# nschejtman/deepLoopCloser

Measured on AMD Instinct MI355X. Metric: query-frames/sec vs N-keyframe DB + top-k recall@1, higher is better.
Workload: dtype bf16; 1 GPU; 1000000 x 4096 bf16 keyframe DB, Q=256, top-20 cosine match, 1 GPU(s); db_rows=1000000, dim=4096, k=20, rows_per_gpu=1000000, pipelined=False, crowded=False

## Files before the change

deeploopcloser_amd/_lib.py:

```python
import ctypes as C
import os

_HERE = os.path.dirname(os.path.abspath(__file__))
LIB_PATH = os.path.join(_HERE, "libdlc_hip.so")

DLC_OK = 0
DLC_ERR_BAD_ARG, DLC_ERR_BAD_SHAPE, DLC_ERR_UNSUPPORTED, DLC_ERR_HIP, DLC_ERR_WORKSPACE = -1, -2, -3, -4, -5
DLC_BF16, DLC_F16, DLC_F32, DLC_F64, DLC_I8, DLC_U8, DLC_I64 = 0, 1, 2, 3, 4, 5, 6
DLC_ACT_NONE, DLC_ACT_SIGMOID, DLC_ACT_RELU = 0, 1, 2
DLC_B_KN, DLC_B_NK = 0, 1
DLC_MAX_K = 128
DLC_MAX_STEP = 8
DLC_MAX_SHIFT = 8
DLC_ABI_VERSION = 20
DLC_SELECT_COOP, DLC_SELECT_NO_HINTS, DLC_SELECT_SERIAL = 1, 2, 4
DLC_PRUNE_ON, DLC_PRUNE_OFF, DLC_PRUNE_KEEP = 0, 1, 2
DLC_SIM_FORCE_F64, DLC_SIM_NO_HOST_SYNC = 1, 2
DLC_MAX_FUSE = 8
DLC_FUSE_NONE, DLC_FUSE_ZSCORE, DLC_FUSE_MINMAX = 0, 1, 2
DLC_FUSE_PLAN_AUTO, DLC_FUSE_PLAN_ROW, DLC_FUSE_PLAN_SLAB = 0, 1, 2
DLC_TRACK_AUTO, DLC_TRACK_RESIDENT, DLC_TRACK_ROWS = 0, 1, 2
DLC_TRACK_RESIDENT_MAX = 8192
DLC_TRACK_JUMP, DLC_TRACK_FROM_NULL, DLC_TRACK_ORIGIN, DLC_TRACK_ABSENT = -1, -2, -3, -128
DLC_TRACK_END_FILTERED, DLC_TRACK_NO_PATH = -2, -2
# ... 104 lines not shown
    "dlc_pca_project_workspace_bytes": (_sz, [_i64, _i64, _int, _int]),
    "dlc_pca_project": (_int, [_vp, _vp, _i64, _i64, _i64, _vp, _int, _vp, _int, _i64, _vp, _vp, _i64, _int, _vp, _sz, _vp]),
    "dlc_pr_cell_counts_workspace_bytes": (_sz, [_i64, _i64, _int]),
    "dlc_pr_cell_counts": (_int, [_vp, _int, _vp, _i64, _i64, _i64, _i64, _i64, _int, _int, _i64, _vp, _i64, _vp, _int, _vp, _vp,
                                  _vp, _sz, _vp]),
    "dlc_positive_rank_rows_workspace_bytes": (_sz, [_i64, _i64]),
    "dlc_positive_rank_rows": (_int, [_vp, _int, _vp, _i64, _i64, _i64, _i64, _i64, _int, _int, _i64, _vp, _i64, _vp, _vp, _vp,
                                      _vp, _sz, _vp]),
    "dlc_l2_normalize_rows": (_int, [_vp, _int, _vp, _i64, _i64, _i64, _int, _int, _vp, _i64, _vp]),
    "dlc_cosine_topk_workspace_bytes": (_sz, [_i64, _i64, _i64, _int]),
    "dlc_cosine_topk": (_int, [_vp, _int, _vp, _i64, _i64, _vp, _i64, _i64, _i64, _int, _i64, _vp, _vp, _vp, _vp, _vp, _vp, _sz,
                              _vp]),
    "dlc_max_row_norm": (_int, [_vp, _int, _vp, _i64, _i64, _i64, _vp, _vp]),
    "dlc_cosine_tau_scale": (_int, [_vp, _int, _vp, _i64, _i64, _i64, _vp, _vp, _vp]),
    "dlc_cosine_topk_older": (_int, [_vp, _int, _vp, _i64, _i64, _vp, _i64, _i64, _i64, _int, _i64, _i64, _vp, _vp, _vp, _vp, _vp,
                                    _vp, _sz, _vp]),
    "dlc_cosine_score_error_bound": (_dbl, [_i64, _i64, _i64, _int]),
    "dlc_cosine_score_error_bound_any_plan": (_dbl, [_i64]),
    "dlc_cosine_score_groups": (_int, [_vp, _int, _vp, _i64, _i64, _vp, _i64, _i64, _i64, _int, _vp, _sz, _vp]),
    "dlc_cosine_select_topk": (_int, [_vp, _int, _vp, _i64, _i64, _vp, _i64, _i64, _i64, _int, _i64, _vp, _vp, _vp, _vp, _vp, _vp,
                                     _sz, _int, _vp]),
    "dlc_cosine_groups_per_query": (_int, [_int]),
    "dlc_cosine_select_groups": (_int, [_vp, _int, _vp, _i64, _i64, _vp, _i64, _i64, _i64, _int, _vp, _sz, _vp, _vp, _int,
                                       _vp]),
    "dlc_cosine_rescore_topk": (_int, [_vp, _int, _vp, _i64, _i64, _vp, _i64, _i64, _i64, _int, _i64, _vp, _vp, _vp, _int,
                                      _vp, _vp, _vp, _vp, _int, _vp]),
    "dlc_cosine_exhaustive_topk": (_int, [_vp, _int, _vp, _i64, _i64, _vp, _i64, _i64, _i64, _int, _i64, _vp, _i64, _dbl,
                                         _vp, _vp, _vp, _vp, _vp, _vp, _sz, _vp]),
    "dlc_topk_merge_strided": (_int, [_vp, _vp, _i64, _vp, _i64, _int, _i64, _int, _vp, _dbl, _vp, _vp, _vp, _vp, _vp, _vp]),
    "dlc_topk_merge": (_int, [_vp, _vp, _vp, _int, _i64, _int, _vp, _vp, _vp, _vp]),
    "dlc_topk_keep_older": (_int, [_vp, _vp, _vp, _i64, _int, _i64, _int, _vp, _vp, _vp]),
    "dlc_cosine_scores_workspace_bytes": (_sz, [_i64, _i64, _i64]),
    "dlc_cosine_scores": (_int, [_vp, _int, _vp, _i64, _i64, _vp, _i64, _i64, _i64, _vp, _i64, _vp, _sz, _vp]),
    "dlc_cosine_score_rows": (_int, [_vp, _int, _vp, _i64, _i64, _vp, _i64, _i64, _i64, _i64, _i64, _vp, _vp, _i64, _vp]),
    "dlc_host_to_device": (_int, [_vp, _vp, _vp, _sz, _vp]),
    "dlc_device_to_host": (_int, [_vp, _vp, _vp, _sz, _vp]),
    "dlc_set_host_threads": (_int, [_vp, _int]),
    "dlc_set_scratch": (_int, [_vp, _vp, _sz]),
    "dlc_set_profiling": (_int, [_vp, _int]),
    "dlc_set_prune_mode": (_int, [_vp, _int]),
    "dlc_cosine_topk_prune_bytes": (_sz, [_i64, _i64, _i64, _int]),
    "dlc_profile_gemm_ms": (_int, [_vp, C.POINTER(_flt), _int]),
}

_lib = None


class DlcError(RuntimeError):
    """A HIP-side failure (DLC_ERR_HIP / DLC_ERR_WORKSPACE) reported by the C ABI."""


def load():
    global _lib
    if _lib is not None:
        return _lib
    if not os.path.exists(LIB_PATH):
        raise ImportError(
            "deeploopcloser_amd: %s is missing -- build it with `python -c 'import __graft_entry__ as g; g.build()'` "
            "or `make -C deeploopcloser_amd/csrc`.  There is no CPU fallback." % LIB_PATH)
    lib = C.CDLL(LIB_PATH)
    for name, (res, args) in SIGNATURES.items():
        fn = getattr(lib, name)
        fn.restype = res
        fn.argtypes = args
    if lib.dlc_abi_version() != DLC_ABI_VERSION:
        raise ImportError("deeploopcloser_amd: %s has ABI %d, these bindings are for ABI %d -- rebuild it"
# ... 14 lines not shown
```

deeploopcloser_amd/csrc/cosine_topk.hip:

```cpp
#include "dlc_internal.h"
#include "lds_dma.h"

#include <algorithm>

namespace {

constexpr int BM = 256;
constexpr int BNQ = 256;
constexpr int BK = 64;
constexpr int NTHREADS = 512;
constexpr int TILE_BYTES = 256 * BK * 2;
constexpr int A_TILE = TILE_BYTES;
constexpr int B_TILE = TILE_BYTES;
#ifndef DLC_A_STAGES
#define DLC_A_STAGES 2
#endif
constexpr int A_STAGES = DLC_A_STAGES;
constexpr int B_RING = A_STAGES * A_TILE;
constexpr int LDS_BYTES = A_STAGES * A_TILE + 2 * B_TILE;
#ifndef DLC_STAGGER_SLEEP
#define DLC_STAGGER_SLEEP 15
#endif
#ifndef DLC_STAGGER_PHASES
#define DLC_STAGGER_PHASES 32
// ... 48 lines not shown
struct alignas(8) HintEntry {
    float r2;
    int id;
};

struct GemmArgs {
    const char* Q;
    const char* DB;
    long long ldq_b;
    long long lddb_b;
    int q;
    long long n;
    int nk;
    float* gmax;
    long long ldg;
    float* tmax;
    long long ldt;
    HintEntry* hint;
    long long ng;
    long long nh;
    float* S;
    long long lds;
    int stagger_mult;
    int stagger_phases;
    int nqb;
    long long ntiles;
    int nsplit;
    int kchunk;
    float* P;
    long long ldp;
    unsigned* bkt;
    unsigned* thr;
    int kt;
};

constexpr int GEMM_GROUPS = 0;
constexpr int GEMM_DENSE = 1;
constexpr int GEMM_PARTIAL = 2;

constexpr int HALF_BYTES = 128 * 128;

#ifndef DLC_A_CACHE_POLICY
#define DLC_A_CACHE_POLICY " nt"
#endif
DLC_DMA_S_FORM(dma_s_stream, DLC_A_CACHE_POLICY)

constexpr int tail_vmcnt_a(int left) {
    const int whole = (left < A_STAGES - 1 ? left : A_STAGES - 1) - 1;
    return 8 * (whole > 0 ? whole : 0) + (left >= A_STAGES ? 4 : 0);
}
constexpr int tail_vmcnt_b(int left) { return left >= 2 ? 8 : 0; }
static_assert(A_STAGES == 2 || A_STAGES == 3, "the database ring is 2 or 3 K tiles deep");
static_assert(A_STAGES != 2 || (tail_vmcnt_a(2) == 4 && tail_vmcnt_a(1) == 0 && tail_vmcnt_a(0) == 0), "2-deep A ring");
static_assert(A_STAGES != 3 || (tail_vmcnt_a(3) == 12 && tail_vmcnt_a(2) == 8 && tail_vmcnt_a(1) == 0 && tail_vmcnt_a(0) == 0),
              "3-deep A ring");

template <typename Tag, int MODE, bool MASKQ>
__global__ __launch_bounds__(NTHREADS, 2) void score_gemm_kernel(GemmArgs p) {
    extern __shared__ __attribute__((aligned(16))) char smem[];
    const int tid = threadIdx.x;
    const int lane = tid & 63;
    const int wid = __builtin_amdgcn_readfirstlane(tid >> 6);
    const int wr = wid >> 2;
    const int wc = wid & 3;
    const unsigned chunk = MODE == GEMM_PARTIAL ? blockIdx.x % (unsigned)p.nsplit : 0u;
    const unsigned wg = MODE == GEMM_PARTIAL ? blockIdx.x / (unsigned)p.nsplit : blockIdx.x;
    const unsigned run = 8u * (unsigned)p.nqb;
    const int j_ = (int)(wg % run);
    const long long tile = (long long)(wg / run) * 8 + (j_ & 7);
    const int qblk = j_ >> 3;
    if (tile >= p.ntiles) return;
    const unsigned lds_base = (unsigned)(unsigned long long)(lptr_t)smem;

    const bool is_a = wid < 4;
    const int ridx = wid & 3;
    const int k_begin = MODE == GEMM_PARTIAL ? (int)chunk * p.kchunk : 0;
    const char* a_base = p.DB + tile * BM * p.lddb_b + (long long)k_begin * 128;
    const char* b_base = p.Q + (long long)qblk * BNQ * p.ldq_b + (long long)k_begin * 128;
    unsigned voff[2][4];
    {
        const int slot = lane & 7;
        const long long arows = p.n - tile * BM;
        const long long brows = (long long)p.q - (long long)qblk * BNQ;
#pragma unroll
        for (int j = 0; j < 4; ++j) {
            const int r = 32 * ridx + 8 * j + (lane >> 3);
#pragma unroll
            for (int h = 0; h < 2; ++h) {
                long long ar = (r >> 6) * 128 + h * 64 + (r & 63);
                if (ar > arows - 1) ar = arows - 1;
                long long br = (r >> 5) * 64 + h * 32 + (r & 31);
                if (br > brows - 1) br = brows - 1;
                voff[h][j] = is_a ? (unsigned)(ar * p.lddb_b + ((slot ^ swz_a(r)) << 4))
                                  : (unsigned)(br * p.ldq_b + ((slot ^ swz_b(r)) << 4));
            }
        }
    }
    const unsigned lds_stage = lds_base + (unsigned)(32 * ridx) * 128;
    const int nk = MODE == GEMM_PARTIAL ? min(p.kchunk, p.nk - k_begin) : p.nk;

    const int i = lane & 15;
    const int kq = lane >> 4;
    const int fa = ((i >> 1) & 1) | ((i >> 2) << 1);
    const int fb = (i >> 1) & 7;
    typedef const __attribute__((address_space(3))) u32x4_t* lds_u4p;
    const lcptr_t lbase = (lcptr_t)(lptr_t)smem;
    const unsigned rdA0_l = (wr * 64 + 16 * (i >> 2) + (i & 3)) * 128 + (((0 + kq) ^ fa) << 4);
    const unsigned rdA1_l = (wr * 64 + 16 * (i >> 2) + (i & 3)) * 128 + (((4 + kq) ^ fa) << 4);
    const unsigned rdB0_l = B_RING + (wc * 32 + i) * 128 + (((0 + kq) ^ fb) << 4);
    const unsigned rdB1_l = B_RING + (wc * 32 + i) * 128 + (((4 + kq) ^ fb) << 4);
    unsigned aoff = 0, boff = 0;
    unsigned rdA0 = rdA0_l, rdA1 = rdA1_l, rdB0 = rdB0_l, rdB1 = rdB1_l;

    f32x4_t acc[8][4];
#pragma unroll
    for (int t = 0; t < 8; ++t)
#pragma unroll
        for (int c = 0; c < 4; ++c) acc[t][c] = (f32x4_t){0.f, 0.f, 0.f, 0.f};
    u32x4_t faX[4], faY[4], fbX[2], fbY[2];

    const bool active = !MASKQ || (qblk * BNQ + wc * 64 < p.q);
#define DLC_READ_A(DST, RD, OFF)                      \
    if (!MASKQ || active) _Pragma("unroll") for (int tt = 0; tt < 4; ++tt)  \
        DST[tt] = *(lds_u4p)(lbase + (RD) + (OFF) + tt * 512)
#define DLC_READ_B(DST, RD, OFF)                      \
    if (!MASKQ || active) _Pragma("unroll") for (int c = 0; c < 2; ++c)     \
        DST[c] = *(lds_u4p)(lbase + (RD) + (OFF) + c * 2048)
#define DLC_MFMA(FA, FB, AH, BH)                                                                     \
    if (!MASKQ || active) do {                                                                       \
        __builtin_amdgcn_s_setprio(1);                                                               \
        _Pragma("unroll") for (int tt = 0; tt < 4; ++tt) _Pragma("unroll") for (int c = 0; c < 2; ++c) \
            acc[(AH) * 4 + tt][(BH) * 2 + c] =                                                       \
                Mfma16<Tag>::run(FA[tt], FB[c], acc[(AH) * 4 + tt][(BH) * 2 + c]);                   \
        __builtin_amdgcn_s_setprio(0);                                                               \
    } while (0)
#define DLC_RELEASE()    \
    DLC_WAIT_LGKM0();    \
    wg_barrier()
#define DLC_ISSUE_A(POS, H, t2)                                                                      \
    do {                                                                                             \
        if (is_a)                                                                                    \
            dma_s_stream(voff[H], a_base + (long long)(t2) * 128, lds_stage + (POS) + (H) * HALF_BYTES); \
    } while (0)
    const bool b_on = !MASKQ || (qblk * BNQ + ridx * 64 < p.q);
#define DLC_ISSUE_B(POS, H, t2)                                                                      \
    do {                                                                                             \
        if (!is_a && b_on)                                                                           \
            dma_s(voff[H], b_base + (long long)(t2) * 128, lds_stage + B_RING + (POS) + (H) * HALF_BYTES); \
    } while (0)
#define DLC_WAIT_TILE(L)                                                                             \
    do {                                                                                             \
        if constexpr (tail_vmcnt_a(L) == tail_vmcnt_b(L)) DLC_WAIT_VMCNT(tail_vmcnt_a(L));           \
        else if (is_a) DLC_WAIT_VMCNT(tail_vmcnt_a(L));                                              \
        else DLC_WAIT_VMCNT(tail_vmcnt_b(L));                                                        \
    } while (0)

    if (MODE != GEMM_PARTIAL && wg < 256) {
        const int steps = (int)((tile >> 3) % p.stagger_phases) * p.stagger_mult;
        for (int s_ = 0; s_ < steps; ++s_) __builtin_amdgcn_s_sleep(DLC_STAGGER_SLEEP);
    }
#pragma unroll
    for (int s_ = 0; s_ < A_STAGES; ++s_) {
        if (s_ < nk) {
            DLC_ISSUE_A(s_ * A_TILE, 1, s_);
            DLC_ISSUE_A(s_ * A_TILE, 0, s_);
        }
    }
    DLC_ISSUE_B(0 * B_TILE, 0, 0);
    DLC_ISSUE_B(0 * B_TILE, 1, 0);
    if (nk > 1) {
        DLC_ISSUE_B(1 * B_TILE, 0, 1);
        DLC_ISSUE_B(1 * B_TILE, 1, 1);
    }
    if (nk == 1) DLC_WAIT_VMCNT(0);
    else if (A_STAGES == 3 && is_a && nk > 2) DLC_WAIT_VMCNT(16);
    else DLC_WAIT_VMCNT(8);
    wg_barrier();
    DLC_READ_A(faX, rdA0, 0);
    DLC_READ_B(fbX, rdB0, 0);

#define DLC_K_TILE(L)                                                                                \
    do {                                                                                             \
        DLC_READ_B(fbY, rdB0, HALF_BYTES);                                                           \
        DLC_MFMA(faX, fbX, 0, 0);                                                            \
        DLC_READ_A(faY, rdA0, HALF_BYTES);                                                           \
        DLC_MFMA(faX, fbY, 0, 1);                                                            \
        DLC_READ_A(faX, rdA1, HALF_BYTES);                                                           \
        DLC_MFMA(faY, fbY, 1, 1);                                                            \
        DLC_RELEASE();                                                      \
        DLC_READ_B(fbY, rdB1, 0);                                                                    \
        if constexpr ((L) >= A_STAGES) DLC_ISSUE_A(aoff, 1, t + A_STAGES);                           \
        DLC_MFMA(faY, fbX, 1, 0);                                                            \
        DLC_RELEASE();                                                                       \
        DLC_READ_B(fbX, rdB1, HALF_BYTES);                                                           \
        if constexpr ((L) >= 2) DLC_ISSUE_B(boff, 0, t + 2);                                         \
        DLC_MFMA(faX, fbY, 1, 0);                                                            \
        DLC_RELEASE();                                                                       \
        DLC_READ_A(faY, rdA1, 0);                                                                    \
        if constexpr ((L) >= 2) DLC_ISSUE_B(boff, 1, t + 2);                                         \
        DLC_MFMA(faX, fbX, 1, 1);                                                            \
        DLC_WAIT_TILE(L);                                           \
        DLC_RELEASE();                                               \
        if constexpr ((L) >= A_STAGES) DLC_ISSUE_A(aoff, 0, t + A_STAGES);                           \
        aoff = aoff == (A_STAGES - 1) * A_TILE ? 0u : aoff + A_TILE;    \
        boff ^= B_TILE;                                                                              \
        rdA0 = rdA0_l + aoff; rdA1 = rdA1_l + aoff; rdB0 = rdB0_l + boff; rdB1 = rdB1_l + boff;      \
        DLC_READ_A(faX, rdA0, 0);                                                                    \
        DLC_MFMA(faY, fbX, 0, 1);                                                            \
        DLC_READ_B(fbX, rdB0, 0);                                                                    \
        DLC_MFMA(faY, fbY, 0, 0);                                                            \
        ++t;                                                                                         \
    } while (0)
    static_assert(tail_vmcnt_a(1) == 0 && tail_vmcnt_b(1) == 0 && tail_vmcnt_a(0) == 0 && tail_vmcnt_b(0) == 0 && A_STAGES >= 2,
                  "DLC_K_TILE(1) serves L = 0 too");
    int t = 0;
    while (t < nk - A_STAGES) DLC_K_TILE(A_STAGES);
    if constexpr (A_STAGES == 3) {
        if (nk > 2) DLC_K_TILE(2);
    }
#pragma unroll 1
    while (t < nk) DLC_K_TILE(1);
    DLC_WAIT_VMCNT(0);
    DLC_WAIT_LGKM0();
#undef DLC_K_TILE
#undef DLC_WAIT_TILE
#undef DLC_ISSUE_A
#undef DLC_ISSUE_B
#undef DLC_READ_A
#undef DLC_READ_B
#undef DLC_MFMA
#undef DLC_RELEASE

    const int lg = lane >> 4;
    if constexpr (MODE == GEMM_PARTIAL) {
        float* part = p.P + (long long)chunk * p.q * p.ldp;
#pragma unroll
        for (int c = 0; c < 4; ++c) {
            const int qidx = qblk * BNQ + wc * 64 + c * 16 + i;
            if (qidx >= p.q) continue;
#pragma unroll
            for (int t = 0; t < 8; ++t) {
                const long long row0 = tile * BM + wr * 128 + (t >> 2) * 64 + 16 * lg + 4 * (t & 3);
                *(f32x4_t*)(part + (long long)qidx * p.ldp + row0) = acc[t][c];
            }
        }
    } else if constexpr (MODE == GEMM_DENSE) {
#pragma unroll
        for (int c = 0; c < 4; ++c) {
// ... 1634 lines not shown
    return w.prune_total - w.total;
}

namespace {

struct MatchCall {
    GemmArgs a;
    WsLayout w;
    bool publish_thr = false;
};

int prepare_match(dlc_ctx* ctx, const char* what, int dtype, const void* Q, int64_t q, int64_t ldq, const void* DB,
                  int64_t n, int64_t lddb, int64_t d, int k, void* workspace, size_t workspace_bytes, MatchCall* mc) {
    int rc = check_operands(ctx, dtype, Q, q, ldq, DB, n, lddb, d);
    if (rc != DLC_OK) return rc;
    if (k < 1 || k > DLC_MAX_K) return dlc::fail(ctx, DLC_ERR_BAD_ARG, "%s: k=%d outside 1..%d", what, k, DLC_MAX_K);
    mc->w = ws_layout(q, n, d, k);
    if (!workspace || workspace_bytes < mc->w.total)
        return dlc::fail(ctx, DLC_ERR_WORKSPACE, "%s: workspace %zu < %zu bytes", what, workspace_bytes, mc->w.total);
    if (((uintptr_t)workspace & 255)) return dlc::fail(ctx, DLC_ERR_BAD_ARG, "%s: workspace must be 256-byte aligned", what);
    char* ws = (char*)workspace;
    GemmArgs& a = mc->a;
    a.Q = (const char*)Q; a.DB = (const char*)DB;
    a.ldq_b = ldq * 2; a.lddb_b = lddb * 2;
    a.q = (int)q; a.n = n; a.nk = (int)(d / BK);
    a.gmax = (float*)(ws + mc->w.gmax); a.ldg = mc->w.ldg;
    a.tmax = (float*)(ws + mc->w.tmax); a.ldt = mc->w.ldt;
    a.hint = (HintEntry*)(ws + mc->w.hint);
    a.ng = dlc::cdiv(n, GROUP); a.nh = dlc::cdiv(n, HALF);
    a.S = nullptr; a.lds = 0;
    a.nsplit = mc->w.sp.nsplit; a.kchunk = mc->w.sp.kchunk;
    a.P = (float*)(ws + mc->w.part); a.ldp = mc->w.ldp;
    a.bkt = nullptr; a.thr = nullptr; a.kt = 0;
    return DLC_OK;
}

inline bool small_direct(const MatchCall& mc, int k) {
    return mc.w.dense && mc.a.n <= (int64_t)FIN_THREADS * SMALL_GPT * GROUP && k + DENSE_ROW_SLACK + 1 <= SMALL_KT_MAX;
}

int run_score(dlc_ctx* ctx, int dtype, MatchCall& mc, hipStream_t st, bool partials_only = false) {
    return dlc::profiled(ctx, st, [&]() -> int {
        return (dtype == DLC_BF16) ? launch_scores<dlc_bf16_tag>(ctx, mc.a, false, st, mc.w.dense, partials_only)
                                   : launch_scores<dlc_f16_tag>(ctx, mc.a, false, st, mc.w.dense, partials_only);
    });
}

FinishArgs finish_args(const MatchCall& mc, int k, int64_t n, int64_t d, int64_t q, int64_t row_offset) {
    const GemmArgs& g = mc.a;
    FinishArgs f{};
    f.tmax = g.tmax; f.ldt = g.ldt; f.nh = (int)g.nh;
    f.gmax = g.gmax; f.ldg = g.ldg; f.ng = g.ng;
    f.kg = mc.w.kg;
    f.Q = g.Q; f.ldq_b = g.ldq_b; f.DB = g.DB; f.lddb_b = g.lddb_b;
    f.n = n; f.d = (int)d; f.k = k; f.row_offset = row_offset;
    f.tau = mc.w.tau;
    f.nq = q;
    return f;
}

template <typename Tag, int THREADS, int RS_UNROLL, int MODE>
int launch_finish(dlc_ctx* ctx, FinishArgs f, int64_t q, bool small_lds, hipStream_t st) {
    size_t dsm = fin_lds_fixed(f.kg);
    f.tv_in_lds = MODE != FIN_RESCORE && !small_lds && !fin_register_path(THREADS, MODE == FIN_GROUPS, f.nh) &&
                  (size_t)f.nh * 4 <= FIN_TV_LDS_MAX;
    if (f.tv_in_lds) dsm += (size_t)f.nh * 4;
    dsm = dlc::align_up(dsm, 16);
    void (*fk)(FinishArgs);
    if constexpr (THREADS == 256) fk = finish_topk_coop_kernel<Tag, RS_UNROLL, MODE>;
    else fk = finish_topk_kernel<Tag, THREADS, RS_UNROLL, MODE>;
    if (dsm > 48 * 1024)
        DLC_HIP_CHECK(ctx, hipFuncSetAttribute((const void*)fk, hipFuncAttributeMaxDynamicSharedMemorySize, (int)dsm));
    hipLaunchKernelGGL(fk, dim3((unsigned)q, (unsigned)(MODE == FIN_RESCORE && f.gparts > 1 ? f.gparts : 1)), dim3(THREADS),
                       dsm, st, f);
// ... 322 lines not shown

extern "C" int dlc_topk_merge(dlc_ctx* ctx, const double* scores_f64, const int64_t* idx, int parts, int64_t q, int k,
                              float* out_scores, double* out_scores_f64, int64_t* out_idx, void* stream) {
    return dlc_topk_merge_strided(ctx, scores_f64, q * k, idx, q * k, parts, q, k, nullptr, 0.0, nullptr, out_scores,
                                  out_scores_f64, out_idx, nullptr, stream);
}

extern "C" size_t dlc_cosine_scores_workspace_bytes(int64_t q, int64_t n, int64_t d) {
    if (q < 1 || n < 1 || d < BK) return 0;
    const SplitPlan sp = split_plan(q, n, d);
    return sp.nsplit > 1 ? dlc::align_up((size_t)sp.nsplit * q * dlc::cdiv(n, BM) * BM * 4, 256) : 0;
}

extern "C" int dlc_cosine_scores(dlc_ctx* ctx, int dtype, const void* Q, int64_t q, int64_t ldq, const void* DB,
                                 int64_t n, int64_t lddb, int64_t d, float* S, int64_t lds, void* workspace,
                                 size_t workspace_bytes, void* stream) {
    int rc = check_operands(ctx, dtype, Q, q, ldq, DB, n, lddb, d);
    if (rc != DLC_OK) return rc;
    if (!S || lds < n) return dlc::fail(ctx, DLC_ERR_BAD_ARG, "cosine_scores: bad output");
    const SplitPlan sp = split_plan(q, n, d);
    const size_t need = dlc_cosine_scores_workspace_bytes(q, n, d);
    if (need && (!workspace || workspace_bytes < need))
        return dlc::fail(ctx, DLC_ERR_WORKSPACE, "cosine_scores: workspace %zu < %zu bytes", workspace_bytes, need);
    if (need && ((uintptr_t)workspace & 255)) return dlc::fail(ctx, DLC_ERR_BAD_ARG, "cosine_scores: workspace must be 256-byte aligned");
    dlc::DeviceGuard guard(ctx->device);
    if (!guard.ok) return dlc::fail(ctx, DLC_ERR_HIP, "hipSetDevice(%d) failed", ctx->device);
    GemmArgs a{};
    a.Q = (const char*)Q; a.DB = (const char*)DB;
    a.ldq_b = ldq * 2; a.lddb_b = lddb * 2;
    a.q = (int)q; a.n = n; a.nk = (int)(d / BK);
    a.S = S; a.lds = lds;
    a.nsplit = sp.nsplit; a.kchunk = sp.kchunk;
    a.P = (float*)workspace; a.ldp = dlc::cdiv(n, BM) * BM;
    return (dtype == DLC_BF16) ? launch_scores<dlc_bf16_tag>(ctx, a, true, (hipStream_t)stream)
                               : launch_scores<dlc_f16_tag>(ctx, a, true, (hipStream_t)stream);
}

extern "C" int dlc_l2_normalize_rows(dlc_ctx* ctx, int src_dtype, const void* src, int64_t n, int64_t d, int64_t lds,
                                     int center, int dst_dtype, void* dst, int64_t ldd, void* stream) {
    if (!ctx) return DLC_ERR_BAD_ARG;
    if (!src || !dst || n < 1 || d < 1 || lds < d || ldd < d)
        return dlc::fail(ctx, DLC_ERR_BAD_ARG, "l2_normalize_rows: bad argument");
    if (ldd % BK) return dlc::fail(ctx, DLC_ERR_BAD_SHAPE, "l2_normalize_rows: ldd=%lld must be a multiple of %d", (long long)ldd, BK);
    if (ldd > 0x7fffffff) return dlc::fail(ctx, DLC_ERR_BAD_SHAPE, "l2_normalize_rows: ldd too large");
    if ((uintptr_t)dst & 3) return dlc::fail(ctx, DLC_ERR_BAD_SHAPE, "l2_normalize_rows: dst must be 4-byte aligned");
    dlc::DeviceGuard guard(ctx->device);
    if (!guard.ok) return dlc::fail(ctx, DLC_ERR_HIP, "hipSetDevice(%d) failed", ctx->device);
    hipStream_t st = (hipStream_t)stream;
    if (src_dtype != DLC_F32 && src_dtype != DLC_F64)
        return dlc::fail(ctx, DLC_ERR_UNSUPPORTED, "l2_normalize_rows: dtype pair %d -> %d", src_dtype, dst_dtype);
    if (dst_dtype != DLC_BF16 && dst_dtype != DLC_F16)
        return dlc::fail(ctx, DLC_ERR_UNSUPPORTED, "l2_normalize_rows: dtype pair %d -> %d", src_dtype, dst_dtype);
    unsigned short* o = (unsigned short*)dst;
    const int vw = src_dtype == DLC_F32 ? 4 : 2;
    const bool aligned = ((uintptr_t)src & 15) == 0 && (lds % vw) == 0 && ((uintptr_t)dst & 7) == 0;
    const int64_t cap_wave = 64 * 4 * vw, cap_block = 256 * 16 * vw;
#define DLC_NORM_REGS(SRC, TAG, TPR)                                                                              \
    hipLaunchKernelGGL((l2_normalize_regs_kernel<SRC, TAG, TPR, 16>), dim3((unsigned)(TPR == 64 ? dlc::cdiv(n, 4) : n)), \
                       dim3(256), 0, st, (const SRC*)src, (long long)lds, (long long)n, (int)d, center, o, (long long)ldd)
#define DLC_NORM(SRC, TAG) \
    hipLaunchKernelGGL((l2_normalize_kernel<SRC, TAG>), dim3((unsigned)n), dim3(256), 0, st, (const SRC*)src, (long long)lds, (int)d, center, o, (long long)ldd)
#define DLC_NORM_PICK(SRC, TAG)                                                   \
    do {                                                                          \
        if (aligned && ldd <= cap_wave) DLC_NORM_REGS(SRC, TAG, 64);              \
        else if (aligned && ldd <= cap_block) DLC_NORM_REGS(SRC, TAG, 256);       \
        else DLC_NORM(SRC, TAG);                                                  \
    } while (0)
    if (src_dtype == DLC_F32 && dst_dtype == DLC_BF16) DLC_NORM_PICK(float, dlc_bf16_tag);
// ... 114 lines not shown
```

deeploopcloser_amd/csrc/dlc_internal.h:

```cpp
#pragma once
#include <hip/hip_runtime.h>
#include <stdint.h>
#include <stdarg.h>
#include <stdio.h>
#include <string.h>
#include <mutex>

#include "../../include/dlc.h"

struct dlc_host_staging;

struct dlc_ctx {
    int device;
    char err[512];
    int profiling;
    long long prof_calls;
    hipEvent_t ev_start[DLC_PROFILE_RING];
    hipEvent_t ev_stop[DLC_PROFILE_RING];
    void* scratch;
    size_t scratch_bytes;
    unsigned long long func_attr_set;
    void* zero_page;
    dlc_host_staging* staging;
    std::mutex* host_lock;
    int host_threads;
    unsigned long long* host_flag;
    hipEvent_t ev_flag;
    int prune_mode;
    int prune_kept;
    const void* prune_id[3];
    long long prune_shape[4];
};

enum {
    DLC_ATTR_GEMM_BASE = 0,
    DLC_ATTR_GEMV_BASE = 16,
    DLC_ATTR_DGEMM_BASE = 24,
    DLC_ATTR_DMA64_BASE = 32,
    DLC_ATTR_PAIR_TILE = 48,
    DLC_ATTR_GRAM_I8 = 49,
    DLC_ATTR_PAIR_FILTER = 50,
    DLC_ATTR_SPLIT_F16 = 51,
    DLC_ATTR_DS_DMA = 52,
    DLC_ATTR_CONV_SPLIT_F16 = 53,
    DLC_ATTR_TRACK_BASE = 54,
};

namespace dlc {

void staging_free(dlc_host_staging* s);

inline int fail(dlc_ctx* ctx, int status, const char* fmt, ...) {
    if (ctx) {
        va_list ap;
        va_start(ap, fmt);
        vsnprintf(ctx->err, sizeof(ctx->err), fmt, ap);
        va_end(ap);
    }
    return status;
}

#define DLC_HIP_CHECK(ctx, expr)                                                              \
    do {                                                                                      \
        hipError_t e__ = (expr);                                                              \
// ... 93 lines not shown
```

deeploopcloser_amd/engine.py:

```python
import collections
import contextlib
import ctypes as C
import weakref

import numpy as np
import torch

from . import _lib as L

_TORCH_TO_DLC = {torch.bfloat16: L.DLC_BF16, torch.float16: L.DLC_F16, torch.float32: L.DLC_F32,
                 torch.float64: L.DLC_F64, torch.int8: L.DLC_I8}
_NAME_TO_TORCH = {"bf16": torch.bfloat16, "bfloat16": torch.bfloat16, "f16": torch.float16, "fp16": torch.float16,
                  "float16": torch.float16, "f32": torch.float32, "float32": torch.float32, "f64": torch.float64,
                  "float64": torch.float64}

SCRATCH_BYTES = 256 << 20
K_STEP = 64


TopK = collections.namedtuple("TopK", "scores idx scores_f64 status")


_RAW_STREAM = getattr(torch._C, "_cuda_getCurrentRawStream", None)

# ... 1563 lines not shown
        self._check(self.lib.dlc_topk_keep_older(self.ctx, _ptr(scores), _ptr(idx), b, kk, int(limit0), int(k), _ptr(o_s),
                                                  _ptr(o_i), self._stream()))
        return o_s, o_i

    def topk_merge(self, scores_f64, idx, out=None, details=False):
        scores_f64, idx = scores_f64.contiguous(), idx.contiguous()
        if scores_f64.dim() != 3 or idx.shape != scores_f64.shape or scores_f64.dtype != torch.float64 or \
                idx.dtype != torch.int64:
            raise ValueError("topk_merge: scores float64 / idx int64 of one shape [parts, Q, k]")
        parts, nq, k = scores_f64.shape
        if out is None:
            o_s = torch.empty((nq, k), dtype=torch.float32, device=self.device)
            o_i = torch.empty((nq, k), dtype=torch.int64, device=self.device)
        else:
            o_s = self._check_out("out[0] (scores)", out[0], (nq, k), torch.float32)
            o_i = self._check_out("out[1] (idx)", out[1], (nq, k), torch.int64)
        o_64 = torch.empty((nq, k), dtype=torch.float64, device=self.device) if details else None
        self._check(self.lib.dlc_topk_merge(self.ctx, _ptr(scores_f64), _ptr(idx), parts, nq, k, _ptr(o_s), _ptr(o_64),
                                             _ptr(o_i), self._stream()))
        return TopK(o_s, o_i, o_64, None) if details else (o_s, o_i)

    def cosine_scores(self, q, db):
        self._check_stored(q, db)
        nq, d = q.shape
        n = db.shape[0]
        s = torch.empty((nq, n), dtype=torch.float32, device=self.device)
        need = self.lib.dlc_cosine_scores_workspace_bytes(nq, n, d)
        ws = self.workspace("scores", need) if need else None
        self._check(self.lib.dlc_cosine_scores(self.ctx, _TORCH_TO_DLC[q.dtype], _ptr(q), nq, q.stride(0), _ptr(db), n,
                                                db.stride(0), d, _ptr(s), s.stride(0), _ptr(ws) if need else None,
                                                need, self._stream()))
        return s

    def cosine_score_rows(self, q, db, limit0=None, limit_step=0, out=None, keys=False, out_keys=None):
        if q.dim() != 2 or db.dim() != 2 or q.dtype != db.dtype or q.dtype not in (torch.bfloat16, torch.float16):
            raise ValueError("cosine_score_rows: q and db must be 2-D, both bf16 or both fp16")
        if q.device != self.device or db.device != self.device:
            raise ValueError("cosine_score_rows: q and db must be on %s" % self.device)
        if q.shape[1] != db.shape[1]:
            raise ValueError("cosine_score_rows: q and db widths differ (%d, %d)" % (q.shape[1], db.shape[1]))
        if q.stride(1) != 1 or db.stride(1) != 1:
            raise ValueError("cosine_score_rows: stored descriptor rows must be contiguous")
        nq, d = q.shape
        n = db.shape[0]
        want_keys = bool(keys) or out_keys is not None
        want_scores = out is not None or not want_keys

        def result(t, dtype, name, fill):
            return self._rows_out("cosine_score_rows: " + name, t, nq, n, dtype, "a %s" % dtype,
                                  None if limit0 is None else fill)

        o_s = result(out, torch.float64, "out", float("nan")) if want_scores else None
        o_k = result(out_keys, torch.int64, "out_keys", -(1 << 63)) if want_keys else None
        both = o_s is not None and o_k is not None
        ret = (o_s, o_k) if both else (o_k if o_k is not None else o_s)
        if nq == 0 or n == 0:
            return ret
        if d == 0:
            raise ValueError("cosine_score_rows: empty descriptors")
        ld_out = (o_s if o_s is not None else o_k).stride(0) if nq > 1 else n
        if both and nq > 1 and o_k.stride(0) != ld_out:
            raise ValueError("cosine_score_rows: out and out_keys must have one row stride (%d, %d)" % (ld_out, o_k.stride(0)))
        self._check(self.lib.dlc_cosine_score_rows(self.ctx, _TORCH_TO_DLC[q.dtype], _ptr(q), nq, q.stride(0), _ptr(db), n,
                                                    db.stride(0), d, *_limits(n, limit0, limit_step),
                                                    _ptr(o_s), _ptr(o_k), ld_out, self._stream()))
        for t in (o_s, o_k):
# ... 34 lines not shown
```

deeploopcloser_amd/matching.py:

```python
import numpy as np
import torch

from .engine import default_engine, torch_dtype


def encode(frames, network):
    return network.transform(frames)


def flatten_frame_descriptors(h, patches=30):
    h = h if isinstance(h, torch.Tensor) else torch.from_numpy(np.asarray(h))
    return h.reshape(h.shape[0] // patches, patches * h.shape[1])


def vlad_frame_descriptors(h, vlad, patches=30):
    return vlad.transform_tensor(h, patches)


class KeyframeDatabase:

    def __init__(self, descriptors, dtype="bf16", center=False, row_offset=0, device=None, stored=False,
                 capacity=None, _norm_bound=None):
        self.engine = default_engine(device)
        self.dtype = torch_dtype(dtype)
        self.center = center
        self.row_offset = int(row_offset)
        self.norm_bound = None
        if stored:
            d = descriptors.to(self.engine.device)
            if d.dtype != self.dtype:
                raise ValueError("stored descriptors have dtype %s, expected %s" % (d.dtype, self.dtype))
            rows = d
            if _norm_bound is not None:
                self.norm_bound = _norm_bound[0]
            elif d.shape[0] > 0 and not self.engine.unit_rows(d):
                self.norm_bound = self.engine.max_row_norm(
                    d, out=torch.full((1,), 1.005, dtype=torch.float32, device=self.engine.device))
        else:
            rows = self.engine.normalize(self._as_float(descriptors), self.dtype, center)
        self._n = rows.shape[0]
        if capacity is not None and capacity > self._n:
            self._store = torch.empty((int(capacity), rows.shape[1]), dtype=self.dtype, device=self.engine.device)
            self._store[:self._n] = rows
        else:
            self._store = rows

    @classmethod
    def empty(cls, dim, capacity=4096, dtype="bf16", center=False, row_offset=0, device=None):
        if dim < 1 or capacity < 1:
            raise ValueError("KeyframeDatabase.empty: dim and capacity must be positive")
        eng = default_engine(device)
        dt = torch_dtype(dtype)
        if dt not in (torch.bfloat16, torch.float16):
            raise ValueError("stored descriptor dtype must be bf16 or fp16")
        none = torch.empty((0, eng.stored_width(dim)), dtype=dt, device=eng.device)
        return cls(none, dtype=dt, center=center, row_offset=row_offset, device=device, stored=True, capacity=capacity)

    def _as_float(self, descriptors):
        x = self.engine.to_device(descriptors)
        if x.dtype not in (torch.float32, torch.float64):
            x = x.to(torch.float32)
        return x

    @property
    def rows(self):
        return self._store[:self._n]

    @property
    def capacity(self):
        return self._store.shape[0]

    def __len__(self):
        return self._n

    def reserve(self, capacity):
        if capacity > self.capacity:
            grown = torch.empty((int(capacity), self._store.shape[1]), dtype=self.dtype, device=self.engine.device)
            grown[:self._n] = self._store[:self._n]
            self._store = grown

    def append(self, descriptors):
        x = self._as_float(descriptors)
        if x.dim() != 2 or self.engine.stored_width(x.shape[1]) != self._store.shape[1]:
            raise ValueError("append: descriptors must be [B, dim] with the database's width")
        b = x.shape[0]
        if self._n + b > self.capacity:
            self.reserve(max(2 * self.capacity, self._n + b))
        self.engine.normalize(x, self.dtype, self.center, out=self._store[self._n:self._n + b])
        first = self.row_offset + self._n
        self._n += b
        return first, first + b

    def prefix(self, n):
        if not 0 <= n <= self._n:
            raise ValueError("prefix: n=%d outside 0..%d" % (n, self._n))
        return KeyframeDatabase(self._store[:n], dtype=self.dtype, center=self.center, row_offset=self.row_offset,
                                device=self.engine.device, stored=True, _norm_bound=(self.norm_bound,))

    def save(self, path):
        np.savez(path, rows_u16=self.rows.view(torch.int16).cpu().numpy().view(np.uint16),
                 dtype=np.array(str(self.dtype).replace("torch.", "")), center=np.array(bool(self.center)),
                 row_offset=np.array(self.row_offset, dtype=np.int64), format=np.array("dlc-keyframes-v1"))

    @classmethod
    def load(cls, path, device=None, row_offset=None):
        z = np.load(path)
        if str(z["format"]) != "dlc-keyframes-v1":
            raise ValueError("%s is not a dlc-keyframes-v1 file" % path)
        dt = torch_dtype(str(z["dtype"]))
        rows = torch.from_numpy(z["rows_u16"].view(np.int16).copy()).view(dt)
        return cls(rows, dtype=dt, center=bool(z["center"]), device=device, stored=True,
                   row_offset=int(z["row_offset"]) if row_offset is None else row_offset)

    def prepare_queries(self, queries):
        x = self.engine.to_device(queries)
        if x.dtype in (torch.bfloat16, torch.float16):
            return x
        return self.engine.normalize(self._as_float(x), self.dtype, self.center)

    def tau_scale(self, q, out=None, stream=None):
        if self.norm_bound is None and self.engine.unit_rows(q):
            return None
        return self.engine.cosine_tau_scale(q, self.norm_bound, out=out, stream=stream)

    def match_topk(self, queries, k, out=None, details=False):
        q = self.prepare_queries(queries)
        return self.engine.match_topk(q, self.rows, k, self.row_offset, out=out, details=details, tau_scale=self.tau_scale(q))

    def match(self, queries):
        return self.engine.cosine_scores(self.prepare_queries(queries), self.rows)
# ... 179 lines not shown
```

include/dlc.h:

```cpp
#ifndef DLC_H_
#define DLC_H_

#include <stddef.h>
#include <stdint.h>

#ifdef __cplusplus
extern "C" {
#endif

#define DLC_ABI_VERSION 20

typedef struct dlc_ctx dlc_ctx;

typedef enum dlc_status {
    DLC_OK = 0,
    DLC_ERR_BAD_ARG = -1,
    DLC_ERR_BAD_SHAPE = -2,
    DLC_ERR_UNSUPPORTED = -3,
    DLC_ERR_HIP = -4,
    DLC_ERR_WORKSPACE = -5
} dlc_status;

typedef enum dlc_dtype {
    DLC_BF16 = 0,
// ... 307 lines not shown
                           const void* DB, int64_t n, int64_t lddb, int64_t d, int k, int64_t row_offset,
                           float* out_scores, double* out_scores_f64, int64_t* out_idx, int32_t* out_status,
                           const float* tau_scale, void* workspace, size_t workspace_bytes, int flags, void* stream);
int dlc_cosine_groups_per_query(int k);
int dlc_cosine_select_groups(dlc_ctx* ctx, int dtype, const void* Q, int64_t q, int64_t ldq,
                             const void* DB, int64_t n, int64_t lddb, int64_t d, int k,
                             void* workspace, size_t workspace_bytes,
                             int32_t* group_ids, float* group_max, int flags, void* stream);
int dlc_cosine_rescore_topk(dlc_ctx* ctx, int dtype, const void* Q, int64_t q, int64_t ldq,
                            const void* DB, int64_t n, int64_t lddb, int64_t d, int k, int64_t row_offset,
                            const int32_t* group_ids, const float* group_max,
                            const float* all_group_max, int parts,
                            double* out_scores_f64, int64_t* out_idx, float* out_bound, const float* tau_scale,
                            int flags, void* stream);
int dlc_cosine_exhaustive_topk(dlc_ctx* ctx, int dtype, const void* Q, int64_t q, int64_t ldq,
                               const void* DB, int64_t n, int64_t lddb, int64_t d, int k, int64_t row_offset,
                               const double* lower, int64_t lower_stride, double tau, const float* tau_scale,
                               int32_t* status, float* out_scores, double* out_scores_f64, int64_t* out_idx,
                               void* workspace, size_t workspace_bytes, void* stream);
int dlc_topk_keep_older(dlc_ctx* ctx, const float* scores, const int64_t* idx, int64_t rows, int kk,
                        int64_t limit0, int k, float* out_scores, int64_t* out_idx, void* stream);
int dlc_topk_merge(dlc_ctx* ctx, const double* scores_f64, const int64_t* idx, int parts, int64_t q, int k,
                   float* out_scores, double* out_scores_f64, int64_t* out_idx, void* stream);
int dlc_topk_merge_strided(dlc_ctx* ctx, const double* scores_f64, int64_t score_part_stride,
                           const int64_t* idx, int64_t idx_part_stride, int parts, int64_t q, int k,
                           const float* bound, double tau, const float* tau_scale,
                           float* out_scores, double* out_scores_f64, int64_t* out_idx, int32_t* out_status,
                           void* stream);
size_t dlc_cosine_scores_workspace_bytes(int64_t q, int64_t n, int64_t d);
int dlc_cosine_scores(dlc_ctx* ctx, int dtype, const void* Q, int64_t q, int64_t ldq,
                      const void* DB, int64_t n, int64_t lddb, int64_t d,
                      float* S, int64_t lds, void* workspace, size_t workspace_bytes, void* stream);

int dlc_cosine_score_rows(dlc_ctx* ctx, int dtype ,
                          const void* Q, int64_t q, int64_t ldq,
                          const void* DB, int64_t n, int64_t lddb, int64_t d,
                          int64_t limit0, int64_t limit_step,
                          double* out_scores, int64_t* out_keys, int64_t ld_out, void* stream);

int dlc_host_to_device(dlc_ctx* ctx, void* dst_device, const void* src_host, size_t bytes, void* stream);
int dlc_device_to_host(dlc_ctx* ctx, void* dst_host, const void* src_device, size_t bytes, void* stream);
int dlc_set_host_threads(dlc_ctx* ctx, int threads);

int dlc_set_scratch(dlc_ctx* ctx, void* scratch, size_t bytes);

#define DLC_PROFILE_RING 256
int dlc_set_profiling(dlc_ctx* ctx, int enabled);
int dlc_profile_gemm_ms(dlc_ctx* ctx, float* out_ms, int capacity);

#ifdef __cplusplus
}
#endif
#endif
```

Before: 128,900 query-frames/s.

## Pre-pack keyframe database into tile-contiguous swizzled layout for GEMM streaming

Adds a one-time pack kernel that rewrites the database into per-(tile, K-step) contiguous 32 KB blocks in exactly the order the LDS DMA loads them. The scoring kernel then reads those blocks with a fixed stride instead of gathering 16-byte pieces from 256 rows spread across the row-major matrix. The aim is more contiguous, better-coalesced HBM reads of the dominant database stream. The cost is a second copy of the database in device memory, a pack pass at build time, and bookkeeping to invalidate the copy on append or growth.

```diff
diff --git a/deeploopcloser_amd/_lib.py b/deeploopcloser_amd/_lib.py
--- a/deeploopcloser_amd/_lib.py
+++ b/deeploopcloser_amd/_lib.py
@@ -160,6 +160,10 @@
     "dlc_topk_keep_older": (_int, [_vp, _vp, _vp, _i64, _int, _i64, _int, _vp, _vp, _vp]),
     "dlc_cosine_scores_workspace_bytes": (_sz, [_i64, _i64, _i64]),
     "dlc_cosine_scores": (_int, [_vp, _int, _vp, _i64, _i64, _vp, _i64, _i64, _i64, _vp, _i64, _vp, _sz, _vp]),
+    "dlc_cosine_pack_bytes": (_sz, [_i64, _i64]),
+    "dlc_cosine_pack_db": (_int, [_vp, _int, _vp, _i64, _i64, _i64, _vp, _vp]),
+    "dlc_cosine_attach_packed": (_int, [_vp, _int, _vp, _i64, _i64, _i64, _vp]),
+    "dlc_cosine_detach_packed": (_int, [_vp, _vp, _vp]),
     "dlc_cosine_score_rows": (_int, [_vp, _int, _vp, _i64, _i64, _vp, _i64, _i64, _i64, _i64, _i64, _vp, _vp, _i64, _vp]),
     "dlc_host_to_device": (_int, [_vp, _vp, _vp, _sz, _vp]),
     "dlc_device_to_host": (_int, [_vp, _vp, _vp, _sz, _vp]),
diff --git a/deeploopcloser_amd/csrc/cosine_topk.hip b/deeploopcloser_amd/csrc/cosine_topk.hip
--- a/deeploopcloser_amd/csrc/cosine_topk.hip
+++ b/deeploopcloser_amd/csrc/cosine_topk.hip
@@ -104,7 +104,19 @@
     unsigned* bkt;
     unsigned* thr;
     int kt;
+    const char* packed;
+    long long packed_tiles;
 };
+
+__device__ __forceinline__ unsigned pack_src_offset(int h, int ridx, int j, int lane, long long arows, long long lddb_b) {
+    const int r = 32 * ridx + 8 * j + (lane >> 3);
+    long long ar = (r >> 6) * 128 + h * 64 + (r & 63);
+    if (ar > arows - 1) ar = arows - 1;
+    return (unsigned)(ar * lddb_b + (((lane & 7) ^ swz_a(r)) << 4));
+}
+__device__ __forceinline__ unsigned pack_dst_offset(int h, int ridx, int j, int lane) {
+    return (unsigned)(((h * 4 + ridx) * 4 + j) * 1024 + lane * 16);
+}
 
 constexpr int GEMM_GROUPS = 0;
 constexpr int GEMM_DENSE = 1;
@@ -147,7 +159,10 @@
     const bool is_a = wid < 4;
     const int ridx = wid & 3;
     const int k_begin = MODE == GEMM_PARTIAL ? (int)chunk * p.kchunk : 0;
-    const char* a_base = p.DB + tile * BM * p.lddb_b + (long long)k_begin * 128;
+    const bool pk = p.packed != nullptr && tile < p.packed_tiles;
+    const char* a_base = pk ? p.packed + (tile * p.nk + k_begin) * (long long)TILE_BYTES
+                            : p.DB + tile * BM * p.lddb_b + (long long)k_begin * 128;
+    const unsigned a_kstride = pk ? TILE_BYTES : 128;
     const char* b_base = p.Q + (long long)qblk * BNQ * p.ldq_b + (long long)k_begin * 128;
     unsigned voff[2][4];
     {
@@ -159,11 +174,9 @@
             const int r = 32 * ridx + 8 * j + (lane >> 3);
 #pragma unroll
             for (int h = 0; h < 2; ++h) {
-                long long ar = (r >> 6) * 128 + h * 64 + (r & 63);
-                if (ar > arows - 1) ar = arows - 1;
                 long long br = (r >> 5) * 64 + h * 32 + (r & 31);
                 if (br > brows - 1) br = brows - 1;
-                voff[h][j] = is_a ? (unsigned)(ar * p.lddb_b + ((slot ^ swz_a(r)) << 4))
+                voff[h][j] = is_a ? (pk ? pack_dst_offset(h, ridx, j, lane) : pack_src_offset(h, ridx, j, lane, arows, p.lddb_b))
                                   : (unsigned)(br * p.ldq_b + ((slot ^ swz_b(r)) << 4));
             }
         }
@@ -209,10 +222,10 @@
 #define DLC_RELEASE()    \
     DLC_WAIT_LGKM0();    \
     wg_barrier()
-#define DLC_ISSUE_A(POS, H, t2)                                                                      \
+#define DLC_ISSUE_A(POS, H, SRC)                                                                     \
     do {                                                                                             \
         if (is_a)                                                                                    \
-            dma_s_stream(voff[H], a_base + (long long)(t2) * 128, lds_stage + (POS) + (H) * HALF_BYTES); \
+            dma_s_stream(voff[H], (SRC), lds_stage + (POS) + (H) * HALF_BYTES);                      \
     } while (0)
     const bool b_on = !MASKQ || (qblk * BNQ + ridx * 64 < p.q);
 #define DLC_ISSUE_B(POS, H, t2)                                                                      \
@@ -234,8 +247,8 @@
 #pragma unroll
     for (int s_ = 0; s_ < A_STAGES; ++s_) {
         if (s_ < nk) {
-            DLC_ISSUE_A(s_ * A_TILE, 1, s_);
-            DLC_ISSUE_A(s_ * A_TILE, 0, s_);
+            DLC_ISSUE_A(s_ * A_TILE, 1, a_base + (long long)s_ * a_kstride);
+            DLC_ISSUE_A(s_ * A_TILE, 0, a_base + (long long)s_ * a_kstride);
         }
     }
     DLC_ISSUE_B(0 * B_TILE, 0, 0);
@@ -261,7 +274,7 @@
         DLC_MFMA(faY, fbY, 1, 1);                                                            \
         DLC_RELEASE();                                                      \
         DLC_READ_B(fbY, rdB1, 0);                                                                    \
-        if constexpr ((L) >= A_STAGES) DLC_ISSUE_A(aoff, 1, t + A_STAGES);                           \
+        if constexpr ((L) >= A_STAGES) DLC_ISSUE_A(aoff, 1, a_next);        \
         DLC_MFMA(faY, fbX, 1, 0);                                                            \
         DLC_RELEASE();                                                                       \
         DLC_READ_B(fbX, rdB1, HALF_BYTES);                                                           \
@@ -273,7 +286,7 @@
         DLC_MFMA(faX, fbX, 1, 1);                                                            \
         DLC_WAIT_TILE(L);                                           \
         DLC_RELEASE();                                               \
-        if constexpr ((L) >= A_STAGES) DLC_ISSUE_A(aoff, 0, t + A_STAGES);                           \
+        if constexpr ((L) >= A_STAGES) { DLC_ISSUE_A(aoff, 0, a_next); a_next += a_kstride; }        \
         aoff = aoff == (A_STAGES - 1) * A_TILE ? 0u : aoff + A_TILE;    \
         boff ^= B_TILE;                                                                              \
         rdA0 = rdA0_l + aoff; rdA1 = rdA1_l + aoff; rdB0 = rdB0_l + boff; rdB1 = rdB1_l + boff;      \
@@ -286,6 +299,7 @@
     static_assert(tail_vmcnt_a(1) == 0 && tail_vmcnt_b(1) == 0 && tail_vmcnt_a(0) == 0 && tail_vmcnt_b(0) == 0 && A_STAGES >= 2,
                   "DLC_K_TILE(1) serves L = 0 too");
     int t = 0;
+    const char* a_next = a_base + (long long)A_STAGES * a_kstride;
     while (t < nk - A_STAGES) DLC_K_TILE(A_STAGES);
     if constexpr (A_STAGES == 3) {
         if (nk > 2) DLC_K_TILE(2);
@@ -1986,6 +2000,7 @@
     a.nsplit = mc->w.sp.nsplit; a.kchunk = mc->w.sp.kchunk;
     a.P = (float*)(ws + mc->w.part); a.ldp = mc->w.ldp;
     a.bkt = nullptr; a.thr = nullptr; a.kt = 0;
+    a.packed = nullptr; a.packed_tiles = 0;
     return DLC_OK;
 }
 
@@ -1993,7 +2008,35 @@
     return mc.w.dense && mc.a.n <= (int64_t)FIN_THREADS * SMALL_GPT * GROUP && k + DENSE_ROW_SLACK + 1 <= SMALL_KT_MAX;
 }
 
+__global__ __launch_bounds__(256) void pack_db_kernel(const char* DB, long long n, long long lddb_b, int nk, char* packed) {
+    const long long tile = blockIdx.x / (unsigned)nk;
+    const int kt = (int)(blockIdx.x % (unsigned)nk);
+    const char* src = DB + tile * BM * lddb_b + (long long)kt * 128;
+    char* dst = packed + (long long)blockIdx.x * TILE_BYTES;
+    const long long arows = n - tile * BM;
+#pragma unroll
+    for (int c = threadIdx.x; c < TILE_BYTES / 16; c += 256) {
+        const int h = c >> 10, ridx = (c >> 8) & 3, j = (c >> 6) & 3, lane = c & 63;
+        const uint4 v = *(const uint4*)(src + pack_src_offset(h, ridx, j, lane, arows, lddb_b));
+        *(uint4*)(dst + pack_dst_offset(h, ridx, j, lane)) = v;
+    }
+}
+
+void use_packed(dlc_ctx* ctx, int dtype, GemmArgs& a) {
+    a.packed = nullptr; a.packed_tiles = 0;
+    std::lock_guard<std::mutex> lk(*ctx->host_lock);
+    for (int i = 0; i < ctx->n_packed; ++i) {
+        const dlc_packed_db& e = ctx->packed[i];
+        if (e.db == (const void*)a.DB && e.dtype == dtype && e.lddb * 2 == a.lddb_b && e.d == (int64_t)a.nk * BK && a.n <= e.n) {
+            a.packed = (const char*)e.packed;
+            a.packed_tiles = a.n / BM;
+            return;
+        }
+    }
+}
+
 int run_score(dlc_ctx* ctx, int dtype, MatchCall& mc, hipStream_t st, bool partials_only = false) {
+    use_packed(ctx, dtype, mc.a);
     return dlc::profiled(ctx, st, [&]() -> int {
         return (dtype == DLC_BF16) ? launch_scores<dlc_bf16_tag>(ctx, mc.a, false, st, mc.w.dense, partials_only)
                                    : launch_scores<dlc_f16_tag>(ctx, mc.a, false, st, mc.w.dense, partials_only);
@@ -2382,8 +2425,57 @@
     a.S = S; a.lds = lds;
     a.nsplit = sp.nsplit; a.kchunk = sp.kchunk;
     a.P = (float*)workspace; a.ldp = dlc::cdiv(n, BM) * BM;
+    use_packed(ctx, dtype, a);
     return (dtype == DLC_BF16) ? launch_scores<dlc_bf16_tag>(ctx, a, true, (hipStream_t)stream)
                                : launch_scores<dlc_f16_tag>(ctx, a, true, (hipStream_t)stream);
+}
+
+extern "C" size_t dlc_cosine_pack_bytes(int64_t n, int64_t d) {
+    if (n < 1 || d < BK || d % BK != 0 || n > 0x7ffffff0ll) return 0;
+    return (size_t)dlc::cdiv(n, BM) * (size_t)(d / BK) * TILE_BYTES;
+}
+
+extern "C" int dlc_cosine_pack_db(dlc_ctx* ctx, int dtype, const void* DB, int64_t n, int64_t lddb, int64_t d, void* packed,
+                                  void* stream) {
+    if (!ctx) return DLC_ERR_BAD_ARG;
+    int rc = check_operands(ctx, dtype, DB, 1, lddb, DB, n, lddb, d);
+    if (rc != DLC_OK) return rc;
+    if (!packed || ((uintptr_t)packed & 255)) return dlc::fail(ctx, DLC_ERR_BAD_ARG, "cosine_pack_db: packed must be 256-byte aligned");
+    const long long blocks = dlc::cdiv(n, BM) * (d / BK);
+    if (blocks > 0x7fffffffll) return dlc::fail(ctx, DLC_ERR_BAD_SHAPE, "cosine_pack_db: %lld blocks exceed the grid limit", blocks);
+    dlc::DeviceGuard guard(ctx->device);
+    if (!guard.ok) return dlc::fail(ctx, DLC_ERR_HIP, "hipSetDevice(%d) failed", ctx->device);
+    hipLaunchKernelGGL(pack_db_kernel, dim3((unsigned)blocks), dim3(256), 0, (hipStream_t)stream, (const char*)DB, (long long)n,
+                       (long long)lddb * 2, (int)(d / BK), (char*)packed);
+    DLC_LAUNCH_CHECK(ctx, "pack_db_kernel");
+    return DLC_OK;
+}
+
+extern "C" int dlc_cosine_attach_packed(dlc_ctx* ctx, int dtype, const void* DB, int64_t n, int64_t lddb, int64_t d,
+                                        const void* packed) {
+    if (!ctx) return DLC_ERR_BAD_ARG;
+    int rc = check_operands(ctx, dtype, DB, 1, lddb, DB, n, lddb, d);
+    if (rc != DLC_OK) return rc;
+    if (!packed || ((uintptr_t)packed & 255)) return dlc::fail(ctx, DLC_ERR_BAD_ARG, "cosine_attach_packed: packed must be 256-byte aligned");
+    std::lock_guard<std::mutex> lk(*ctx->host_lock);
+    int slot = ctx->n_packed;
+    for (int i = 0; i < ctx->n_packed; ++i) {
+        const dlc_packed_db& e = ctx->packed[i];
+        if (e.db == DB && e.n == n && e.lddb == lddb && e.d == d && e.dtype == dtype) slot = i;
+    }
+    if (slot == DLC_MAX_PACKED) return dlc::fail(ctx, DLC_ERR_BAD_ARG, "cosine_attach_packed: %d databases are attached already", DLC_MAX_PACKED);
+    ctx->packed[slot] = dlc_packed_db{DB, packed, n, lddb, d, dtype};
+    if (slot == ctx->n_packed) ctx->n_packed++;
+    return DLC_OK;
+}
+
+extern "C" int dlc_cosine_detach_packed(dlc_ctx* ctx, const void* DB, const void* packed) {
+    if (!ctx) return DLC_ERR_BAD_ARG;
+    std::lock_guard<std::mutex> lk(*ctx->host_lock);
+    for (int i = ctx->n_packed - 1; i >= 0; --i)
+        if (ctx->packed[i].db == DB && (!packed || ctx->packed[i].packed == packed))
+            ctx->packed[i] = ctx->packed[--ctx->n_packed];
+    return DLC_OK;
 }
 
 extern "C" int dlc_l2_normalize_rows(dlc_ctx* ctx, int src_dtype, const void* src, int64_t n, int64_t d, int64_t lds,
diff --git a/deeploopcloser_amd/csrc/dlc_internal.h b/deeploopcloser_amd/csrc/dlc_internal.h
--- a/deeploopcloser_amd/csrc/dlc_internal.h
+++ b/deeploopcloser_amd/csrc/dlc_internal.h
@@ -9,6 +9,14 @@
 #include "../../include/dlc.h"
 
 struct dlc_host_staging;
+
+struct dlc_packed_db {
+    const void* db;
+    const void* packed;
+    int64_t n, lddb, d;
+    int dtype;
+};
+constexpr int DLC_MAX_PACKED = 16;
 
 struct dlc_ctx {
     int device;
@@ -30,6 +38,8 @@
     int prune_kept;
     const void* prune_id[3];
     long long prune_shape[4];
+    dlc_packed_db packed[DLC_MAX_PACKED];
+    int n_packed;
 };
 
 enum {
diff --git a/deeploopcloser_amd/engine.py b/deeploopcloser_amd/engine.py
--- a/deeploopcloser_amd/engine.py
+++ b/deeploopcloser_amd/engine.py
@@ -1619,6 +1619,36 @@
                                                 need, self._stream()))
         return s
 
+    def _check_db_rows(self, who, db):
+        if db.dim() != 2 or db.dtype not in (torch.bfloat16, torch.float16) or db.stride(1) != 1 or db.device != self.device:
+            raise ValueError("%s: stored rows [n, d] (bf16 / fp16, contiguous rows) on %s" % (who, self.device))
+
+    def pack_bytes(self, n, d):
+        return int(self.lib.dlc_cosine_pack_bytes(int(n), int(d)))
+
+    def pack_database(self, db, out=None):
+        self._check_db_rows("pack_database", db)
+        need = self.pack_bytes(db.shape[0], db.shape[1])
+        if need == 0:
+            raise ValueError("pack_database: [%d, %d] rows cannot be packed" % tuple(db.shape))
+        if out is None:
+            out = torch.empty((need,), dtype=torch.uint8, device=self.device)
+        else:
+            self._check_out("out", out, (need,), torch.uint8)
+        self._check(self.lib.dlc_cosine_pack_db(self.ctx, _TORCH_TO_DLC[db.dtype], _ptr(db), db.shape[0], db.stride(0),
+                                                 db.shape[1], _ptr(out), self._stream()))
+        return out
+
+    def attach_packed(self, db, packed):
+        self._check_db_rows("attach_packed", db)
+        self._check_out("packed", packed, (self.pack_bytes(db.shape[0], db.shape[1]),), torch.uint8)
+        self._check(self.lib.dlc_cosine_attach_packed(self.ctx, _TORCH_TO_DLC[db.dtype], _ptr(db), db.shape[0], db.stride(0),
+                                                       db.shape[1], _ptr(packed)))
+
+    def detach_packed(self, db_ptr, packed_ptr=None):
+        if getattr(self, "ctx", None):
+            self._check(self.lib.dlc_cosine_detach_packed(self.ctx, C.c_void_p(db_ptr), C.c_void_p(packed_ptr)))
+
     def cosine_score_rows(self, q, db, limit0=None, limit_step=0, out=None, keys=False, out_keys=None):
         if q.dim() != 2 or db.dim() != 2 or q.dtype != db.dtype or q.dtype not in (torch.bfloat16, torch.float16):
             raise ValueError("cosine_score_rows: q and db must be 2-D, both bf16 or both fp16")
diff --git a/deeploopcloser_amd/matching.py b/deeploopcloser_amd/matching.py
--- a/deeploopcloser_amd/matching.py
+++ b/deeploopcloser_amd/matching.py
@@ -1,3 +1,5 @@
+import os
+
 import numpy as np
 import torch
 
@@ -19,8 +21,10 @@
 
 class KeyframeDatabase:
 
+    PACK_MIN_BYTES = 256 << 20
+
     def __init__(self, descriptors, dtype="bf16", center=False, row_offset=0, device=None, stored=False,
-                 capacity=None, _norm_bound=None):
+                 capacity=None, packed=None, _norm_bound=None):
         self.engine = default_engine(device)
         self.dtype = torch_dtype(dtype)
         self.center = center
@@ -44,6 +48,56 @@
             self._store[:self._n] = rows
         else:
             self._store = rows
+        self._packed = None
+        self._packed_db_ptr = None
+        if self._want_packed(packed, capacity is not None):
+            self._build_packed()
+
+    def _want_packed(self, packed, growing):
+        need = self.engine.pack_bytes(self._n, self._store.shape[1]) if self._n > 0 else 0
+        if need == 0 or packed is False:
+            return False
+        if packed is True:
+            return True
+        if growing:
+            return False
+        env = os.environ.get("DLC_PACK_DB", "")
+        if env in ("0", "1"):
+            return env == "1"
+        if self._n * self._store.shape[1] * self._store.element_size() <= self.PACK_MIN_BYTES:
+            return False
+        dev = self.engine.device
+        free = torch.cuda.mem_get_info(dev)[0] + torch.cuda.memory_reserved(dev) - torch.cuda.memory_allocated(dev)
+        return free >= 2 * need
+
+    def _build_packed(self):
+        rows = self.rows
+        self._packed = self.engine.pack_database(rows)
+        self.engine.attach_packed(rows, self._packed)
+        self._packed_db_ptr = rows.data_ptr()
+
+    @property
+    def packed(self):
+        return self._packed is not None
+
+    def repack(self):
+        if self._packed is not None:
+            self.engine.pack_database(self.rows, out=self._packed)
+
+    def _drop_packed(self):
+        if self._packed is not None:
+            self.engine.detach_packed(self._packed_db_ptr, self._packed.data_ptr())
+            self._packed = None
+            self._packed_db_ptr = None
+
+    def close(self):
+        self._drop_packed()
+
+    def __del__(self):
+        try:
+            self._drop_packed()
+        except Exception:
+            pass
 
     @classmethod
     def empty(cls, dim, capacity=4096, dtype="bf16", center=False, row_offset=0, device=None):
@@ -75,6 +129,7 @@
 
     def reserve(self, capacity):
         if capacity > self.capacity:
+            self._drop_packed()
             grown = torch.empty((int(capacity), self._store.shape[1]), dtype=self.dtype, device=self.engine.device)
             grown[:self._n] = self._store[:self._n]
             self._store = grown
@@ -84,6 +139,7 @@
         if x.dim() != 2 or self.engine.stored_width(x.shape[1]) != self._store.shape[1]:
             raise ValueError("append: descriptors must be [B, dim] with the database's width")
         b = x.shape[0]
+        self._drop_packed()
         if self._n + b > self.capacity:
             self.reserve(max(2 * self.capacity, self._n + b))
         self.engine.normalize(x, self.dtype, self.center, out=self._store[self._n:self._n + b])
@@ -95,7 +151,7 @@
         if not 0 <= n <= self._n:
             raise ValueError("prefix: n=%d outside 0..%d" % (n, self._n))
         return KeyframeDatabase(self._store[:n], dtype=self.dtype, center=self.center, row_offset=self.row_offset,
-                                device=self.engine.device, stored=True, _norm_bound=(self.norm_bound,))
+                                device=self.engine.device, stored=True, packed=False, _norm_bound=(self.norm_bound,))
 
     def save(self, path):
         np.savez(path, rows_u16=self.rows.view(torch.int16).cpu().numpy().view(np.uint16),
diff --git a/include/dlc.h b/include/dlc.h
--- a/include/dlc.h
+++ b/include/dlc.h
@@ -363,6 +363,13 @@
                       const void* DB, int64_t n, int64_t lddb, int64_t d,
                       float* S, int64_t lds, void* workspace, size_t workspace_bytes, void* stream);
 
+size_t dlc_cosine_pack_bytes(int64_t n, int64_t d);
+int dlc_cosine_pack_db(dlc_ctx* ctx, int dtype, const void* DB, int64_t n, int64_t lddb, int64_t d, void* packed,
+                       void* stream);
+int dlc_cosine_attach_packed(dlc_ctx* ctx, int dtype, const void* DB, int64_t n, int64_t lddb, int64_t d,
+                             const void* packed);
+int dlc_cosine_detach_packed(dlc_ctx* ctx, const void* DB, const void* packed);
+
 int dlc_cosine_score_rows(dlc_ctx* ctx, int dtype ,
                           const void* Q, int64_t q, int64_t ldq,
                           const void* DB, int64_t n, int64_t lddb, int64_t d,
```

Result: no change. 130,400 query-frames/s, median of 6 (+1.1%).
